# Justin-Huber/SfM-project

Measured on AMD Instinct MI355X. Metric: verified matches/sec (match+RANSAC), higher is better.
Workload: dtype int8 MFMA -> exact int32 (K1), f32 (K2); 1 GPU; cfg4: all 124750 unordered pairs of 500 synthetic images x 4096 128-D u8 SIFT-like descriptors; L2 match (mutual cross check + ratio 4/5) + 8-point RANSAC 4096 hyp/pair (seed 42, Sampson 1 px^2, min 15 inliers); launches of <= 131072 pairs; n_img=500, k=4096, n_hyp=4096, pairs_total=124750, pairs_rank0=124750, launches_rank0=1, parallelism=pair-sharded dp1

## Files before the change

### sfm-project_amd/csrc/match_l2fr.hip

```cpp
#include <algorithm>
#include <climits>
#include <cstdlib>

#include "l2fr_records.h"
#include "match_common.h"

namespace {

typedef int v4i __attribute__((ext_vector_type(4)));
typedef int v16i __attribute__((ext_vector_type(16)));
typedef __attribute__((address_space(3))) void lds_void;
typedef const __attribute__((address_space(1))) void gbl_void;

constexpr int D = 128;
#ifndef L2FR_WAVES
#define L2FR_WAVES 8
#endif
constexpr int WAVES = L2FR_WAVES;
constexpr int SCAN_THREADS = 64 * WAVES;
#ifndef L2FR_QT
#define L2FR_QT 4
#endif
constexpr int QT = L2FR_QT;
constexpr int QB = WAVES * QT * 32;
constexpr int SCAN_MIN_WAVES = 8 / QT;
#ifndef L2FR_CHUNK
#define L2FR_CHUNK 256
#endif
constexpr int CHUNK = L2FR_CHUNK;
constexpr int GROUP = 256;
constexpr int NT = CHUNK / 32;
constexpr int NK = D / 32;
constexpr int SLOTS = D / 16;
constexpr int PIECES = CHUNK * D / 1024 / WAVES;
constexpr int RPP = 1024 / D;
constexpr int KALIGN = CHUNK > GROUP ? CHUNK : GROUP;
constexpr int KMAX = 4096;
constexpr int PAD_INIT = -(1 << 30);
constexpr int E_VALID = l2fr::E_NONE;
static_assert(D == l2fr::REC_D && KMAX == l2fr::REC_KMAX, "l2fr_records.h is sized for D and KMAX");
typedef unsigned long long rec8;

enum : unsigned char { ST_DROP = 0, ST_CAND = 1, ST_SLOW = 2, ST_PASS = 3 };

__device__ __forceinline__ int swz(int row) { return (row >> 1) & 7; }

__device__ __forceinline__ void top2_insert(int& tb, int& ts, int x, int y) {
    const int med = max(min(tb, x), min(max(tb, x), y));
#ifndef L2FR_NO_ASM_MAX3
    int top;
    asm("v_max3_i32 %0, %1, %2, %3" : "=v"(top) : "v"(tb), "v"(x), "v"(y), "v"(med));
#else
    const int top = max(max(x, y), tb);
#endif
    ts = max(ts, med);
    tb = top;
}

__device__ __forceinline__ int dot128(const uint4* x, const uint4* y) {
    int s = 0;
#pragma unroll
    for (int k = 0; k < 8; ++k) {
        const uint4 u = x[k], v = y[k];
        s = __builtin_amdgcn_sdot4((int)u.x, (int)v.x, s, false);
        s = __builtin_amdgcn_sdot4((int)u.y, (int)v.y, s, false);
        s = __builtin_amdgcn_sdot4((int)u.z, (int)v.z, s, false);
        s = __builtin_amdgcn_sdot4((int)u.w, (int)v.w, s, false);
    }
    return s;
}

__device__ __forceinline__ void prep_one(int img, int j, const uint8_t* __restrict__ desc,
                                         const int32_t* __restrict__ n_kp, int k_max, int k_pad,
                                         int32_t* __restrict__ norm, int32_t* __restrict__ cinit,
                                         uint8_t* __restrict__ zero_row,
                                         uint4* __restrict__ desc_i8) {
    if (img == 0 && j < D) zero_row[j] = 0;
    if (j >= k_pad) return;
    int nv = 0;
    if (j < k_max) {
        const uint4* p = (const uint4*)(desc + ((size_t)img * k_max + j) * D);
        uint4* o8 = desc_i8 + ((size_t)img * k_max + j) * SLOTS;
#pragma unroll
        for (int q = 0; q < SLOTS; ++q) {
            const uint4 v = p[q];
            const uint4 x = make_uint4(v.x ^ 0x80808080u, v.y ^ 0x80808080u, v.z ^ 0x80808080u,
                                       v.w ^ 0x80808080u);
            o8[q] = x;
            nv = __builtin_amdgcn_sdot4((int)x.x, (int)x.x, nv, false);
            nv = __builtin_amdgcn_sdot4((int)x.y, (int)x.y, nv, false);
            nv = __builtin_amdgcn_sdot4((int)x.z, (int)x.z, nv, false);
            nv = __builtin_amdgcn_sdot4((int)x.w, (int)x.w, nv, false);
        }
    }
    const size_t o = (size_t)img * k_pad + j;
    norm[o] = nv;
    cinit[o] = (j < n_kp[img]) ? -((nv + 1) >> 1) : PAD_INIT;
}

constexpr int REC_R = 4;

#ifndef L2FR_UNIT
#define L2FR_UNIT 2
#endif
constexpr int UNIT = L2FR_UNIT;
__device__ void build_units(const int32_t* __restrict__ pairs, int n_pairs, int n_img,
                            const int32_t* __restrict__ n_kp, int4* __restrict__ uinfo,
                            int32_t* __restrict__ n_units, int* lds) {
    int* cur = lds;
    int* fu = lds + n_img;
    int* ru = lds + 2 * n_img + 1;
    __shared__ int ftot;
    const int tid = threadIdx.x;
    for (int i = tid; i < n_img; i += 1024) cur[i] = 0;
    __syncthreads();
    auto live = [&](int a, int b) { return n_kp[a] > 0 && n_kp[b] > 0; };
    for (int p = tid; p < n_pairs; p += 1024)
        if (live(pairs[2 * p], pairs[2 * p + 1])) atomicAdd(&cur[pairs[2 * p]], 1);
    __syncthreads();
    if (tid == 0) {
        int f = 0, r = 0;
        for (int i = 0; i < n_img; ++i) {
            const int c = cur[i];
            fu[i] = f;
            ru[i] = r;
            f += c / UNIT;
            r += (c % UNIT) != 0;
            cur[i] = 0;
        }
        fu[n_img] = f;
        ru[n_img] = r;
        ftot = f;
        *n_units = f + r;
    }
    __syncthreads();
    for (int t = tid; t < ru[n_img] * UNIT; t += 1024) uinfo[(size_t)ftot * UNIT + t] = make_int4(-1, 0, 0, 0);
    __syncthreads();
    for (int p = tid; p < n_pairs; p += 1024) {
        const int a = pairs[2 * p], b = pairs[2 * p + 1];
        if (!live(a, b)) continue;
        const int k = atomicAdd(&cur[a], 1);
        const int nf = UNIT * (fu[a + 1] - fu[a]);
        const int u = k < nf ? fu[a] + k / UNIT : ftot + ru[a];
        const int jj = k < nf ? k % UNIT : k - nf;
        uinfo[(size_t)u * UNIT + jj] = jj ? make_int4(p, b, n_kp[b], 0)
                                          : make_int4(p, a, b, n_kp[a] | (n_kp[b] << 16));
    }
}

__device__ void order_block(int ob, const int32_t* __restrict__ pairs, int n_pairs, int n_img,
                            int32_t* __restrict__ order,
                            int2* __restrict__ rng, int32_t* __restrict__ n_rng,
                            const int32_t* __restrict__ n_kp, int4* __restrict__ rinfo,
                            int4* __restrict__ sinfo_f, int unit_blk, int4* __restrict__ uinfo,
                            int32_t* __restrict__ n_units, int* hist) {
    if (ob == unit_blk) {
        build_units(pairs, n_pairs, n_img, n_kp, uinfo, n_units, hist);
        return;
    }
    const int tid = threadIdx.x;
    for (int i = tid; i < n_img; i += 1024) hist[i] = 0;
    __syncthreads();
    for (int p = tid; p < n_pairs; p += 1024) atomicAdd(&hist[pairs[2 * p + 1]], 1);
    __syncthreads();
    int* roff = hist + n_img;
    if (tid == 0) {
        int off = 0, nr = 0;
        for (int i = 0; i < n_img; ++i) {
            const int c = hist[i];
            roff[i] = nr;
            nr += (c + REC_R - 1) / REC_R;
            hist[i] = off;
            off += c;
        }
        n_rng[0] = nr;
        n_rng[1] = 0;
    }
    __syncthreads();
    for (int i = tid; i < n_img; i += 1024) {
        const int c = (i + 1 < n_img ? hist[i + 1] : n_pairs) - hist[i];
        for (int k = 0; k < c; k += REC_R)
            rng[roff[i] + k / REC_R] = make_int2(hist[i] + k, min(REC_R, c - k));
    }
    __syncthreads();
    for (int p = tid; p < n_pairs; p += 1024) {
        const int a = pairs[2 * p], b = pairs[2 * p + 1];
        const int slot = atomicAdd(&hist[b], 1);
        order[slot] = p;
        sinfo_f[slot] = make_int4(p, a, b, n_kp[a] | (n_kp[b] << 16));
    }
    __threadfence_block();
    __syncthreads();
    const int nr = *n_rng;
    for (int r = tid; r < nr; r += 1024) {
        const int2 g = rng[r];
#pragma unroll
        for (int e = 0; e < REC_R; ++e) {
            int4 v = make_int4(-1, 0, 0, 0);
            if (e < g.y) {
                const int p = order[g.x + e], a = pairs[2 * p], b = pairs[2 * p + 1];
                v = make_int4(p, a, b, n_kp[a] | (n_kp[b] << 16));
            }
            rinfo[(size_t)r * REC_R + e] = v;
        }
    }
}

__global__ __launch_bounds__(1024) void l2fr_setup_kernel(
    int n_prep, int bpi, const uint8_t* __restrict__ desc, const int32_t* __restrict__ n_kp,
    int k_max, int k_pad, int32_t* __restrict__ norm, int32_t* __restrict__ cinit,
    uint8_t* __restrict__ zero_row, uint4* __restrict__ desc_i8, const int32_t* __restrict__ pairs,
    int n_pairs, int n_img, int32_t* __restrict__ order_f,
    int2* __restrict__ rng, int32_t* __restrict__ n_rng, int4* __restrict__ rinfo,
    int4* __restrict__ sinfo_f, int unit_blk, int4* __restrict__ uinfo,
    int32_t* __restrict__ n_units) {
    extern __shared__ int hist[];
    const int b = (int)blockIdx.x;
    if (b < n_prep) {
        const int img = b / bpi;
        prep_one(img, (b - img * bpi) * 1024 + (int)threadIdx.x, desc, n_kp, k_max, k_pad, norm,
                 cinit, zero_row, desc_i8);
        return;
    }
    order_block(b - n_prep, pairs, n_pairs, n_img, order_f, rng, n_rng, n_kp, rinfo,
                sinfo_f, unit_blk, uinfo, n_units, hist);
}

__device__ __forceinline__ unsigned char classify(int e1, int e2, long long A, int rnum, int rden,
                                                  long long max_dist) {
    const long long d1lo = max(A - 2LL * e1 - 1, 0LL);
    const long long d2hi = e2 > E_VALID ? A - 2LL * e2 : sfm::DIST_INF;
    if (!sfm::ratio_ok(d1lo, d2hi, rnum, rden, true) || (max_dist >= 0 && !(d1lo < max_dist)))
        return ST_DROP;
    return (e2 == e1) ? ST_SLOW : ST_CAND;
}

struct FwdCls {
    const int32_t* norm;
    int rnum, rden;
    long long max_dist;
    rec8* fwd;
    uint8_t* cls;
};

#ifdef L2FR_CLOCK
constexpr int L2FR_CLOCK_SLOTS = 1 << 16;
constexpr int L2FR_CLOCK_W = 24;
__device__ unsigned long long g_l2fr_clock[L2FR_CLOCK_W * L2FR_CLOCK_SLOTS];
#define L2FR_STAMP(i, v) \
    if (!REV && tid == 0 && bid < L2FR_CLOCK_SLOTS) g_l2fr_clock[L2FR_CLOCK_W * (size_t)bid + (i)] = (v)
#else
#define L2FR_STAMP(i, v)
#endif

template <bool REV>
__device__ __forceinline__ void scan_body(
    const unsigned bid, const unsigned n_bid, const int n_list,
    const uint8_t* __restrict__ desc, const int32_t* __restrict__ n_kp, int k_max, int k_pad,
    const int32_t* __restrict__ cinit, const uint8_t* __restrict__ zero_row,
    const int32_t* __restrict__ pairs, int n_qblk, const int32_t* __restrict__ pair_order,
    const int4* __restrict__ sinfo, int n_blk, const int4* __restrict__ qlist,
    const int32_t* __restrict__ qcount, int4* __restrict__ out, FwdCls fc,
    const int32_t* __restrict__ n_units) {
    __shared__ __attribute__((aligned(16))) unsigned char lds0[CHUNK * D + CHUNK * 4];
    __shared__ __attribute__((aligned(16))) unsigned char lds1[CHUNK * D + CHUNK * 4];

    int p, qi, ti, nq, nb, qb;
    int p2 = -1, ti2 = 0, nb2 = 0;
    int pos = 0, kk = 0;
    if (!REV && n_units) {
        const int nu = *n_units;
        const int u8 = (nu + 7) >> 3;
        const int l = (int)(bid >> 3);
        qb = u8 > 0 ? l / u8 : n_qblk;
        pos = (l - qb * u8) * 8 + (int)(bid & 7);
        if (qb >= n_qblk || pos >= nu) return;
        const int4 u = sinfo[(size_t)UNIT * pos];
        asm volatile("" : : "s"(u.x), "s"(u.y), "s"(u.z), "s"(u.w));
        p = u.x;
        qi = u.y;
        ti = u.z;
        nq = u.w & 0xFFFF;
        nb = u.w >> 16;
    } else if (REV) {
        qb = (int)bid / n_list;
        p = pair_order[(int)bid - qb * n_list];
        qi = pairs[2 * p + 1];
        ti = pairs[2 * p];
        nq = qcount[p];
        nb = n_kp[ti];
    } else {
        const int ppx = (int)(n_bid >> 3) / n_qblk;
        const int l = (int)(bid >> 3);
        const int pos = (int)(bid & 7) * ppx + l % ppx;
        qb = l / ppx;
        if (pos >= n_blk) return;
        const int4 u = sinfo[pos];
        asm volatile("" : : "s"(u.x), "s"(u.y), "s"(u.z), "s"(u.w));
        p = u.x;
        qi = u.y;
        ti = u.z;
        nq = u.w & 0xFFFF;
        nb = u.w >> 16;
    }
    if (qb * QB >= nq || nb <= 0) return;
    const int tid = threadIdx.x, wave = tid >> 6, lane = tid & 63, h = lane >> 5, r32 = lane & 31;
    L2FR_STAMP(0, __builtin_amdgcn_s_memrealtime());

    const uint8_t* db = desc + (size_t)ti * k_max * D;
    const int32_t* cib = cinit + (size_t)ti * k_pad;
    int n_chunk = (nb + CHUNK - 1) / CHUNK;
    const uint8_t* db2 = desc;
    const int32_t* cib2 = cinit;
    auto find_next = [&]() {
        p2 = -1;
        if (REV || !n_units || ++kk >= UNIT) return;
        const int4 v = sinfo[(size_t)UNIT * pos + kk];
        p2 = v.x;
        ti2 = v.y;
        nb2 = v.z;
        db2 = desc + (size_t)ti2 * k_max * D;
        cib2 = cinit + (size_t)ti2 * k_pad;
    };
    find_next();

    auto stage = [&](const uint8_t* sdb, const int32_t* scib, int snb, int ch, unsigned char* dst) {
#pragma unroll
        for (int i = 0; i < PIECES; ++i) {
            const int piece = wave * PIECES + i;
            const int row = piece * RPP + lane / SLOTS;
            const int slot = (lane % SLOTS) ^ swz(row);
            const int j = ch * CHUNK + row;
            const uint8_t* src = (j < snb) ? sdb + (size_t)j * D + slot * 16 : zero_row + slot * 16;
            __builtin_amdgcn_global_load_lds((gbl_void*)src, (lds_void*)(dst + piece * 1024), 16, 0, 0);
        }
        if (tid < CHUNK / 4) {
            const int32_t* src = scib + ch * CHUNK + tid * 4;
            __builtin_amdgcn_global_load_lds((gbl_void*)src, (lds_void*)(dst + CHUNK * D + wave * 1024),
                                             16, 0, 0);
        }
    };
    auto stage_next = [&](int ch, unsigned char* dst) {
        if (ch + 1 < n_chunk) stage(db, cib, nb, ch + 1, dst);
        else if (p2 >= 0) stage(db2, cib2, nb2, 0, dst);
    };

    const int qbase = qb * QB + wave * QT * 32;
    const bool active = qbase < nq;
    const uint8_t* da = desc + (size_t)qi * k_max * D;

    auto emit = [&](int e, int e1, int e2, int t) {
        if (REV) {
            out[(size_t)p * k_pad + e] = make_int4(e1, e2, t, 0);
        } else {
            fc.fwd[(size_t)p * k_pad + e] = l2fr::pack_fwd(e1, e2, t);
            const unsigned char st =
                classify(e1, e2, fc.norm[(size_t)qi * k_pad + e], fc.rnum, fc.rden, fc.max_dist);
            fc.cls[(size_t)p * k_pad + e] =
                st == ST_CAND ? (uint8_t)t : (st == ST_SLOW ? l2fr::CLS_SLOW : l2fr::CLS_DROP);
        }
    };

#if L2FR_MFMA16
    constexpr int QS = 2 * QT;
    const int g4 = lane >> 4, r16 = lane & 15;
    v4i bq[QS][2];
    int tb[QS], ts[QS], t1[QS];
#pragma unroll
    for (int c = 0; c < QS; ++c) {
        const int e = qbase + c * 16 + r16;
        int row = -1;
        if (e < nq) row = REV ? qlist[(size_t)p * k_pad + e].y : e;
        const v4i* src = (const v4i*)((row >= 0) ? da + (size_t)row * D + 32 * g4 : zero_row + 32 * g4);
        bq[c][0] = src[0];
        bq[c][1] = src[1];
        tb[c] = INT_MIN; ts[c] = INT_MIN; t1[c] = 0;
    }
    v4i acc[QS][2];
    auto process = [&](int ch, const unsigned char* cur, unsigned char* nxt) __attribute__((always_inline)) {
        stage_next(ch, nxt);
        const int nt = min(NT, (nb - ch * CHUNK + 31) >> 5);
        if (active) {
            const int* Ci = (const int*)(cur + CHUNK * D);
            auto load_tile = [&](int tt, v4i (&af)[2][2], v4i (&init)[2]) {
#pragma unroll
                for (int u = 0; u < 2; ++u) {
                    const int row = tt * 32 + 16 * u + r16;
                    const int sw = swz(row);
#pragma unroll
                    for (int s = 0; s < 2; ++s)
#ifdef L2FR_ABL_NOLDS
                        af[u][s] = bq[(tt + u + s) & (QS - 1)][s];
#else
                        af[u][s] = *(const v4i*)(cur + row * D + (((2 * g4 + s) ^ sw) << 4));
#endif
#ifdef L2FR_ABL_NOLDS
                    init[u] = v4i{tt, u, tt, u};
#else
                    init[u] = *(const v4i*)(Ci + tt * 32 + 16 * u + 4 * g4);
#endif
                }
            };
            v4i af[2][2], init[2];
            load_tile(0, af, init);
            for (int tt = 0; tt < nt; ++tt) {
                const int gt = ch * NT + tt;
#ifndef L2FR_NO_MPRIO
                __builtin_amdgcn_s_setprio(1);
#endif
#pragma unroll
                for (int s = 0; s < 2; ++s)
#pragma unroll
                    for (int u = 0; u < 2; ++u)
#pragma unroll
                        for (int c = 0; c < QS; ++c)
                            acc[c][u] = __builtin_amdgcn_mfma_i32_16x16x64_i8(
                                af[u][s], bq[c][s], s == 0 ? init[u] : acc[c][u], 0, 0, 0);
#ifndef L2FR_NO_MPRIO
                __builtin_amdgcn_s_setprio(0);
#endif
                if (tt + 1 < nt) load_tile(tt + 1, af, init);
#pragma unroll
                for (int c = 0; c < QS; ++c) {
                    const int o = tb[c];
#ifdef L2FR_ABL_NOEPI
                    tb[c] = max(tb[c], acc[c][0][0] ^ acc[c][1][3]);
#else
#pragma unroll
                    for (int u = 0; u < 2; ++u) {
                        top2_insert(tb[c], ts[c], acc[c][u][0], acc[c][u][1]);
                        top2_insert(tb[c], ts[c], acc[c][u][2], acc[c][u][3]);
                    }
#endif
                    t1[c] = (tb[c] != o) ? gt : t1[c];
                }
            }
        }
    };
#else
    v4i bq[QT][NK];
    int tb[QT], ts[QT], t1[QT];
#pragma unroll
    for (int c = 0; c < QT; ++c) {
        const int e = qbase + c * 32 + r32;
        int row = -1;
        if (e < nq) row = REV ? qlist[(size_t)p * k_pad + e].y : e;
        const v4i* src = (const v4i*)((row >= 0) ? da + (size_t)row * D + (D / 2) * h
                                                 : zero_row + (D / 2) * h);
#pragma unroll
        for (int s = 0; s < NK; ++s) bq[c][s] = src[s];
        tb[c] = INT_MIN; ts[c] = INT_MIN; t1[c] = 0;
    }

    v16i acc[QT];
    auto epi_all = [&](int gt) {
#pragma unroll
        for (int u = 0; u < QT; ++u) {
            const int o = tb[u];
#ifdef L2FR_ABL_NOEPI
            tb[u] = max(tb[u], acc[u][0] ^ acc[u][15]);
#else
#pragma unroll
            for (int r = 0; r < 16; r += 2) top2_insert(tb[u], ts[u], acc[u][r], acc[u][r + 1]);
#endif
            t1[u] = (tb[u] != o) ? gt : t1[u];
        }
    };

    auto process = [&](int ch, const unsigned char* cur, unsigned char* nxt) __attribute__((always_inline)) {
        stage_next(ch, nxt);
        const int nt = min(NT, (nb - ch * CHUNK + 31) >> 5);
        if (active) {
            const int* Ci = (const int*)(cur + CHUNK * D);
            auto load_tile = [&](int tt, v4i (&af)[NK], v16i& init) {
                const int row = tt * 32 + r32;
                const int sw = swz(row);
#pragma unroll
                for (int s = 0; s < NK; ++s)
#ifdef L2FR_ABL_NOLDS
                    af[s] = bq[(tt + s) & (QT - 1)][s];
#else
                    af[s] = *(const v4i*)(cur + row * D + ((((SLOTS / 2) * h + s) ^ sw) << 4));
#endif
#pragma unroll
                for (int g = 0; g < 4; ++g) {
#ifdef L2FR_ABL_NOLDS
                    const v4i cv = v4i{tt, g, tt, g};
#else
                    const v4i cv = *(const v4i*)(Ci + tt * 32 + 8 * g + 4 * h);
#endif
                    init[4 * g + 0] = cv.x; init[4 * g + 1] = cv.y;
                    init[4 * g + 2] = cv.z; init[4 * g + 3] = cv.w;
                }
            };
            v4i af[NK];
            v16i init;
            load_tile(0, af, init);
            for (int tt = 0; tt < nt; ++tt) {
                const int gt = ch * NT + tt;
#ifndef L2FR_NO_MPRIO
                __builtin_amdgcn_s_setprio(1);
#endif
#pragma unroll
                for (int s = 0; s < NK; ++s)
#pragma unroll
                    for (int c = 0; c < QT; ++c)
                        acc[c] = __builtin_amdgcn_mfma_i32_32x32x32_i8(af[s], bq[c][s],
                                                                        s == 0 ? init : acc[c], 0, 0, 0);
#ifndef L2FR_NO_MPRIO
                __builtin_amdgcn_s_setprio(0);
#endif
                if (tt + 1 < nt) load_tile(tt + 1, af, init);
                epi_all(gt);
            }
        }
    };
#endif

    auto epilogue = [&]() {
#if L2FR_MFMA16
#pragma unroll
        for (int c = 0; c < QS; ++c) {
            int e1 = tb[c], e2 = ts[c], t = t1[c];
#pragma unroll
            for (int m = 16; m <= 32; m <<= 1) {
                const int P1 = __shfl_xor(e1, m), P2 = __shfl_xor(e2, m), PT = __shfl_xor(t, m);
                e2 = max(min(e1, P1), max(e2, P2));
                t = e1 > P1 ? t : (P1 > e1 ? PT : min(t, PT));
                e1 = max(e1, P1);
            }
            const int e = qbase + c * 16 + r16;
            if (g4 == 0 && e < nq) emit(e, e1, e2, t);
            tb[c] = INT_MIN; ts[c] = INT_MIN; t1[c] = 0;
        }
#else
#pragma unroll
        for (int c = 0; c < QT; ++c) {
            const int P1 = __shfl_xor(tb[c], 32), P2 = __shfl_xor(ts[c], 32),
                      PT = __shfl_xor(t1[c], 32);
            const int e1 = max(tb[c], P1);
            const int e2 = max(min(tb[c], P1), max(ts[c], P2));
            const int t = tb[c] > P1 ? t1[c] : (P1 > tb[c] ? PT : min(t1[c], PT));
            const int e = qbase + c * 32 + r32;
            if (h == 0 && e < nq) emit(e, e1, e2, t);
            tb[c] = INT_MIN; ts[c] = INT_MIN; t1[c] = 0;
        }
#endif
    };

    if (n_chunk > 0) stage(db, cib, nb, 0, lds0);
    __syncthreads();
    L2FR_STAMP(1, __builtin_amdgcn_s_memrealtime());
    L2FR_STAMP(2, __builtin_amdgcn_s_memtime());
    auto run_pair = [&](unsigned char* s0, unsigned char* s1) __attribute__((always_inline)) {
        for (int ch = 0; ch < n_chunk; ch += 2) {
            process(ch, s0, s1);
            __syncthreads();
            if (ch < 16) L2FR_STAMP(3 + ch, __builtin_amdgcn_s_memrealtime());
            if (ch + 1 < n_chunk) process(ch + 1, s1, s0);
            __syncthreads();
            if (ch + 1 < 16) L2FR_STAMP(4 + ch, __builtin_amdgcn_s_memrealtime());
        }
    };
    int g = 0;
    for (;;) {
        if (g & 1)
            run_pair(lds1, lds0);
        else
            run_pair(lds0, lds1);
        g += n_chunk;
        L2FR_STAMP(19, __builtin_amdgcn_s_memtime());
        L2FR_STAMP(20, __builtin_amdgcn_s_memrealtime());
        if (active) epilogue();
        if (p2 < 0) break;
        p = p2;
        ti = ti2;
        nb = nb2;
        db = db2;
        cib = cib2;
        n_chunk = (nb + CHUNK - 1) / CHUNK;
        find_next();
    }
#ifdef L2FR_CLOCK
    L2FR_STAMP(21, __builtin_amdgcn_s_memrealtime());
    L2FR_STAMP(22, (unsigned)__builtin_amdgcn_s_getreg((31 << 11) | 4));
    L2FR_STAMP(23, (unsigned)__builtin_amdgcn_s_getreg((15 << 11) | 20));
#endif
}

__global__ __launch_bounds__(SCAN_THREADS, SCAN_MIN_WAVES) void l2fr_scan_fwd_kernel(
    const uint8_t* __restrict__ desc, const int32_t* __restrict__ n_kp, int k_max, int k_pad,
    const int32_t* __restrict__ cinit, const uint8_t* __restrict__ zero_row,
    const int32_t* __restrict__ pairs, int n_qblk, const int4* __restrict__ sinfo, int n_blk,
    FwdCls fc, const int32_t* __restrict__ n_units) {
    scan_body<false>(blockIdx.x, gridDim.x, 0, desc, n_kp, k_max, k_pad, cinit, zero_row, pairs, n_qblk,
                     nullptr, sinfo, n_blk, nullptr, nullptr, nullptr, fc, n_units);
}

constexpr int REV_GRID = 1024;
__global__ __launch_bounds__(SCAN_THREADS, SCAN_MIN_WAVES) void l2fr_scan_rev_kernel(
    const uint8_t* __restrict__ desc, const int32_t* __restrict__ n_kp, int k_max, int k_pad,
    const int32_t* __restrict__ cinit, const uint8_t* __restrict__ zero_row,
    const int32_t* __restrict__ pairs, int n_qblk, const int32_t* __restrict__ flist,
    const int32_t* __restrict__ n_flag, const int4* __restrict__ qlist,
    const int32_t* __restrict__ qcount, int4* __restrict__ out) {
    const int nl = *n_flag;
    for (unsigned u = blockIdx.x; u < (unsigned)(nl * n_qblk); u += gridDim.x) {
        scan_body<true>(u, 0, nl, desc, n_kp, k_max, k_pad, cinit, zero_row, pairs, n_qblk, flist,
                        nullptr, 0, qlist, qcount, out, FwdCls{}, nullptr);
        __syncthreads();
    }
}

struct Top2 { long long b1; int j1; long long b2; };

__device__ __forceinline__ Top2 top2_merge(Top2 x, Top2 y) {
    const bool xf = (x.b1 < y.b1) || (x.b1 == y.b1 && x.j1 < y.j1);
    Top2 r;
    r.b1 = xf ? x.b1 : y.b1;
    r.j1 = xf ? x.j1 : y.j1;
    r.b2 = min(min(x.b2, y.b2), xf ? y.b1 : x.b1);
    return r;
}

__device__ Top2 exact_row_scan(const uint4* qrow, const uint8_t* db, const int32_t* normb, int nb,
                               int qnorm, Top2* red) {
    const int tid = threadIdx.x;
    uint4 x[SLOTS];
#pragma unroll
    for (int s = 0; s < SLOTS; ++s) x[s] = qrow[s];
    Top2 m{sfm::DIST_INF, INT_MAX, sfm::DIST_INF};
    for (int j = tid; j < nb; j += 256) {
        const int dot = dot128(x, (const uint4*)(db + (size_t)j * D));
        const long long d = (long long)qnorm + normb[j] - 2LL * dot;
        m = top2_merge(m, Top2{d, j, sfm::DIST_INF});
    }
    red[tid] = m;
    __syncthreads();
    for (int s = 128; s > 0; s >>= 1) {
        if (tid < s) red[tid] = top2_merge(red[tid], red[tid + s]);
        __syncthreads();
    }
    const Top2 r = red[0];
    __syncthreads();
    return r;
}

__device__ __forceinline__ int compact_rec(bool keep, int4 rec, int base, int* wsum, int4* dst) {
    const int tid = threadIdx.x, lane = tid & 63, wave = tid >> 6;
    const unsigned long long bal = __ballot(keep);
    const int pre = __popcll(bal & ((1ull << lane) - 1ull));
    if (lane == 0) wsum[wave] = __popcll(bal);
    __syncthreads();
    int off = 0, tot = 0;
    for (int w = 0; w < 4; ++w) {
        const int s = wsum[w];
        off += (w < wave) ? s : 0;
        tot += s;
    }
    if (keep) dst[base + off + pre] = rec;
    __syncthreads();
    return base + tot;
}

#ifndef L2FR_REC_SB
#define L2FR_REC_SB 2
#endif
constexpr int REC_SB = L2FR_REC_SB;
__global__ __launch_bounds__(256, REC_SB > 2 ? 2 : 3) void l2fr_recover_mfma_kernel(
    const uint8_t* __restrict__ desc, int k_max, int k_pad, const int32_t* __restrict__ norm,
    const int32_t* __restrict__ cinit, const int4* __restrict__ rinfo,
    const int32_t* __restrict__ n_rng, const rec8* __restrict__ fwd,
    const uint8_t* __restrict__ cls, int rnum, int rden, long long max_dist,
    rec8* __restrict__ qst) {
    __shared__ unsigned short clist[REC_R * KMAX];
    __shared__ __attribute__((aligned(16))) int gini[GROUP];
    __shared__ unsigned char gpar[GROUP];
    __shared__ unsigned long long wlo[4], whi[4];
    __shared__ int toff[9];
    const int ngrp = k_pad / GROUP;
    const int ri = (int)(blockIdx.x / ngrp), grp = (int)(blockIdx.x % ngrp), tid = threadIdx.x;
    if (ri >= *n_rng) return;
    const int wave = tid >> 6, lane = tid & 63, h = lane >> 5, r32 = lane & 31;
    int4 pi[REC_R];
#pragma unroll
    for (int e = 0; e < REC_R; ++e) pi[e] = rinfo[(size_t)ri * REC_R + e];
    const int b = pi[0].z, nb = pi[0].w >> 16;
    const int ntiles = (nb + 31) >> 5, tg = grp * 8;
    if (nb <= 0 || tg >= ntiles) return;
    const uint8_t* db = desc + (size_t)b * k_max * D;

    uint4 cv[REC_R];
#pragma unroll
    for (int e = 0; e < REC_R; ++e) {
        cv[e] = make_uint4(0xFFFFFFFFu, 0xFFFFFFFFu, 0xFFFFFFFFu, 0xFFFFFFFFu);
        if (pi[e].x >= 0 && tid * 16 < (pi[e].w & 0xFFFF))
            cv[e] = ((const uint4*)(cls + (size_t)pi[e].x * k_pad))[tid];
    }
    v4i af[2][NK];
#pragma unroll
    for (int u = 0; u < 2; ++u) {
        const int row = (tg + 2 * wave + u) * 32 + r32;
#pragma unroll
        for (int s = 0; s < NK; ++s)
            af[u][s] = row < nb ? *(const v4i*)(db + (size_t)row * D + 64 * h + 16 * s) : v4i{0, 0, 0, 0};
    }
    {
        const size_t o = (size_t)b * k_pad + tg * 32 + tid;
        gini[tid] = cinit[o];
        gpar[tid] = (unsigned char)(norm[o] & 1);
    }
    unsigned msk[REC_R];
    unsigned long long lo = 0, hi = 0;
    const unsigned g8 = 0x01010101u * ((unsigned)grp << 3);
#pragma unroll
    for (int e = 0; e < REC_R; ++e) {
        const int na = pi[e].x >= 0 ? (pi[e].w & 0xFFFF) : 0;
        const unsigned cw[4] = {cv[e].x, cv[e].y, cv[e].z, cv[e].w};
        unsigned m = 0;
#pragma unroll
        for (int k = 0; k < 4; ++k) {
            const unsigned t = (cw[k] ^ g8) & 0xF8F8F8F8u;
            const unsigned nz = ((t & 0x7F7F7F7Fu) + 0x7F7F7F7Fu) | t;
            const unsigned z = ~nz & 0x80808080u;
            m |= (((z >> 7) & 1u) | ((z >> 14) & 2u) | ((z >> 21) & 4u) | ((z >> 28) & 8u)) << (4 * k);
        }
        const int lim = na - tid * 16;
        m &= lim >= 16 ? 0xFFFFu : (lim <= 0 ? 0u : (1u << lim) - 1u);
        msk[e] = m;
        for (unsigned mm = m; mm; mm &= mm - 1) {
            const int k = __builtin_ctz(mm);
            const unsigned c = (cw[k >> 2] >> (8 * (k & 3))) & 7u;
            const unsigned long long one = 1ull << (16 * (c & 3));
            if (c & 4) hi += one; else lo += one;
        }
    }
    unsigned long long plo = lo, phi = hi;
#pragma unroll
    for (int d = 1; d < 64; d <<= 1) {
        const unsigned long long vl = __shfl_up(plo, d), vh = __shfl_up(phi, d);
        if (lane >= d) { plo += vl; phi += vh; }
    }
    if (lane == 63) { wlo[wave] = plo; whi[wave] = phi; }
    __syncthreads();
    unsigned long long blo = 0, bhi = 0, tlo = 0, thi = 0;
#pragma unroll
    for (int w = 0; w < 4; ++w) {
        blo += w < wave ? wlo[w] : 0ull;
        bhi += w < wave ? whi[w] : 0ull;
        tlo += wlo[w];
        thi += whi[w];
    }
    unsigned long long slo = 0, shi = 0;
    {
        int o = 0;
#pragma unroll
        for (int t = 0; t < 8; ++t) {
            const unsigned long long tot = t < 4 ? tlo : thi, bef = t < 4 ? blo : bhi,
                                     mine = t < 4 ? plo - lo : phi - hi;
            const int sh = 16 * (t & 3);
            const unsigned long long v =
                (unsigned long long)(o + (int)((bef >> sh) & 0xFFFF) + (int)((mine >> sh) & 0xFFFF)) << sh;
// ... 347 lines not shown
#pragma unroll
    for (int i = 0; i < TAIL_NQ; ++i) {
        const int4 w4 = *(const int4*)wcnt[i];
        const int ww[4] = {w4.x, w4.y, w4.z, w4.w};
        int off = M;
#pragma unroll
        for (int w = 0; w < 4; ++w) {
            off += w < wave ? ww[w] : 0;
            M += ww[w];
        }
        const unsigned long long bal = __ballot((outm >> i) & 1u);
        if ((outm >> i) & 1u) {
            const int o = off + __popcll(bal & ((1ull << lane) - 1ull));
            const l2fr::Res r = l2fr::unpack_res(raw[i]);
            om[2 * o] = i * 256 + tid;
            om[2 * o + 1] = r.j1;
            od[o] = r.d1;
        }
    }
    if (tid == 0) {
        out_count[p] = M;
        if (stats) atomicAdd(&stats[0], 1ull);
    }
}

__global__ __launch_bounds__(256) void l2fr_final_kernel(
    const uint8_t* __restrict__ desc, const int32_t* __restrict__ n_kp, int k_max, int k_pad,
    const int32_t* __restrict__ norm, const int32_t* __restrict__ cinit,
    const int32_t* __restrict__ pairs, const int4* __restrict__ surv,
    const int32_t* __restrict__ scount, const int4* __restrict__ rev,
    const int32_t* __restrict__ flist, const int32_t* __restrict__ n_flag,
    int32_t* __restrict__ out_count, int32_t* __restrict__ out_match,
    int32_t* __restrict__ out_dist) {
    __shared__ int wsum[8];
    __shared__ int amb[256];
    __shared__ int namb;
    __shared__ unsigned char keepx[256];
    __shared__ long long redd[256];
    __shared__ int redq[256];
    const int tid = threadIdx.x, nl = *n_flag;
    for (int li = blockIdx.x; li < nl; li += gridDim.x) {
    const int p = flist[li];
    const int a = pairs[2 * p], b = pairs[2 * p + 1];
    const int na = n_kp[a];
    const int S = scount[p];
    const int4* sv = surv + (size_t)p * k_pad;
    const int4* rv = rev + (size_t)p * k_pad;
    const int32_t* na_norm = norm + (size_t)a * k_pad;
    const int32_t* nb_norm = norm + (size_t)b * k_pad;
    const int32_t* ca = cinit + (size_t)a * k_pad;
    const uint8_t* da = desc + (size_t)a * k_max * D;
    const uint4* dbv = (const uint4*)(desc + (size_t)b * k_max * D);
    int32_t* om = out_match + (size_t)p * k_max * 2;
    int32_t* od = out_dist + (size_t)p * k_max;
    int base = 0;
    for (int k0 = 0; k0 < S; k0 += 256) {
        const int k = k0 + tid;
        int4 s = make_int4(0, 0, 0, 0);
        bool keep = false;
        if (tid == 0) namb = 0;
        __syncthreads();
        if (k < S) {
            s = sv[k];
            const int4 r = rv[k];
            const int dot = (int)(((long long)na_norm[s.x] + nb_norm[s.y] - s.z) >> 1);
            const int ep = dot + ca[s.x];
            keep = (ep == r.x) && (r.y < r.x);
            if (ep == r.x && r.y == r.x) amb[atomicAdd(&namb, 1)] = tid;
        }
        keepx[tid] = keep;
        __syncthreads();
        const int nam = namb;
        for (int i = 0; i < nam; ++i) {
            const int who = amb[i];
            const int4 e = sv[k0 + who];
            uint4 y[SLOTS];
#pragma unroll
            for (int u = 0; u < SLOTS; ++u) y[u] = dbv[(size_t)e.y * SLOTS + u];
            long long bd = sfm::DIST_INF;
            int bq = INT_MAX;
            for (int q = tid; q < na; q += 256) {
                const int dot = dot128((const uint4*)(da + (size_t)q * D), y);
                const long long d = (long long)na_norm[q] + nb_norm[e.y] - 2LL * dot;
                if (d < bd) { bd = d; bq = q; }
            }
            redd[tid] = bd; redq[tid] = bq;
            __syncthreads();
            for (int st = 128; st > 0; st >>= 1) {
                if (tid < st) {
                    const long long od2 = redd[tid + st];
                    const int oq = redq[tid + st];
                    if (od2 < redd[tid] || (od2 == redd[tid] && oq < redq[tid])) {
                        redd[tid] = od2; redq[tid] = oq;
                    }
                }
                __syncthreads();
            }
            if (tid == 0) keepx[who] = (redq[0] == e.x);
            __syncthreads();
        }
        keep = keepx[tid] != 0 && k < S;
        base = sfm::compact256(keep, s.x, s.y, s.z, base, wsum, om, od);
    }
    if (tid == 0) out_count[p] = base;
    }
}

__global__ void l2fr_dump_kernel(const int32_t* __restrict__ n_kp, const int32_t* __restrict__ pairs,
                                 int k_max, int k_pad, const int4* __restrict__ rec,
                                 const rec8* __restrict__ fwd8,
                                 const int32_t* __restrict__ cnt, int32_t* __restrict__ out_count,
                                 int32_t* __restrict__ out_match, int32_t* __restrict__ out_dist) {
    const int p = blockIdx.x;
    const int n = cnt ? cnt[p] : n_kp[pairs[2 * p]];
    for (int i = threadIdx.x; i < n; i += blockDim.x) {
        int4 r;
        if (rec) {
            r = rec[(size_t)p * k_pad + i];
        } else {
            const l2fr::Fwd f = l2fr::unpack_fwd(fwd8[(size_t)p * k_pad + i]);
            r = make_int4(f.e1, f.e2, f.tile, 0);
        }
        out_match[((size_t)p * k_max + i) * 2] = r.x;
        out_match[((size_t)p * k_max + i) * 2 + 1] = r.y;
        out_dist[(size_t)p * k_max + i] = r.z;
    }
    if (threadIdx.x == 0) out_count[p] = n;
}

}

int sfm_match_l2fr_launch(sfm_ctx* ctx, const uint8_t* desc, const int32_t* n_kp, int32_t n_img,
                          int32_t k_max, const int32_t* pairs, int32_t n_pairs,
                          const sfm_match_params* prm, int32_t* out_count, int32_t* out_match,
                          int32_t* out_dist) {
    hipStream_t st = ctx->stream;
    if (k_max == 0) {
        SFM_HIP_CHECK(hipMemsetAsync(out_count, 0, sizeof(int32_t) * n_pairs, st));
        return SFM_OK;
    }
    const int k_pad = (int)sfm::align_up((size_t)k_max, KALIGN);
    SFM_REQUIRE(k_pad <= KMAX, "sfm_match_batch: L2 matcher needs k_max <= 4096");
    const int n_qblk = (k_max + QB - 1) / QB;
    const size_t tab = (size_t)n_img * k_pad * sizeof(int32_t);
    const size_t recb = (size_t)n_pairs * k_pad * sizeof(int4);
    const size_t cntb = sfm::align_up(sizeof(int32_t) * (size_t)n_pairs, 256);
    const size_t descb = sfm::align_up((size_t)n_img * k_max * D, 256);
    const size_t ordb = sfm::align_up(sizeof(int32_t) * (size_t)n_pairs, 256);
    const size_t clsb = sfm::align_up((size_t)n_pairs * k_pad, 256);
    const int n_rng_max = n_pairs / REC_R + n_img + 1;
    const size_t rngb = sfm::align_up(sizeof(int2) * (size_t)n_rng_max, 256);
    const size_t rinfob = sizeof(int4) * (size_t)n_rng_max * REC_R;
    const size_t sinfob = sfm::align_up(sizeof(int4) * (size_t)n_pairs, 256);
    const size_t uinfob = sfm::align_up(UNIT * sizeof(int4) * (size_t)n_pairs, 256);
    char* ws = (char*)sfm::workspace(ctx, 256 + 2 * tab + 2 * recb + cntb + descb + ordb + clsb +
                                              256 + rngb + rinfob + 256 + sinfob + uinfob + 256 +
                                              cntb);
    if (!ws) return SFM_ERR_NOMEM;
    char* w = ws;
    uint8_t* zero_row = (uint8_t*)w; w += 256;
    int32_t* norm = (int32_t*)w; w += tab;
    int32_t* cinit = (int32_t*)w; w += tab;
    int4* surv = (int4*)w; w += recb;
    int4* rev = (int4*)w; w += recb;
    rec8* fwd = (rec8*)rev;
    rec8* qst = fwd + (size_t)n_pairs * k_pad;
    int32_t* scount = (int32_t*)w; w += cntb;
    uint8_t* desc_i8 = (uint8_t*)w; w += descb;
    int32_t* ord_f = (int32_t*)w; w += ordb;
    uint8_t* cls = (uint8_t*)w; w += clsb;
    int32_t* n_rng = (int32_t*)w; w += 256;
    int32_t* n_flag = n_rng + 1;
    int2* rng = (int2*)w; w += rngb;
    int4* rinfo = (int4*)w; w += rinfob;
    int4* sinfo_f = (int4*)sfm::align_up((size_t)w, 256);
    int4* uinfo = (int4*)((char*)sinfo_f + sinfob);
    int32_t* n_units = (int32_t*)((char*)uinfo + uinfob);
    int32_t* flist = (int32_t*)((char*)n_units + 256);
    static const bool units_env = [] {
        const char* e = getenv("SFM_L2FR_UNITS");
        return !(e && e[0] == '0');
    }();
    const bool units = units_env && (3 * (size_t)n_img + 2) * sizeof(int) <= 65536;
    const int ppx = (n_pairs + 7) / 8;
    const int n_blk = n_pairs;
    const int grid = 8 * ppx * n_qblk;
    const bool mutual = prm->cross_check == SFM_XC_MUTUAL;

    const int unit_blk = units ? 1 : -1;
    const int bpi = (k_pad + 1023) / 1024, n_prep = bpi * n_img;
    hipLaunchKernelGGL(l2fr_setup_kernel, dim3(n_prep + 1 + (units ? 1 : 0)), dim3(1024),
                       ((units ? 3 : 2) * (size_t)n_img + 2) * sizeof(int), st, n_prep, bpi, desc, n_kp,
                       k_max, k_pad, norm, cinit, zero_row, (uint4*)desc_i8, pairs, n_pairs, n_img,
                       ord_f, rng, n_rng, rinfo, sinfo_f, unit_blk, uinfo, n_units);
    SFM_HIP_CHECK(hipGetLastError());
    const FwdCls fc{norm, prm->ratio_num, prm->ratio_den, (long long)prm->max_dist, fwd, cls};
    hipLaunchKernelGGL(l2fr_scan_fwd_kernel, dim3(grid), dim3(SCAN_THREADS), 0, st, desc_i8, n_kp, k_max,
                       k_pad, cinit, zero_row, pairs, n_qblk, (const int4*)(units ? uinfo : sinfo_f),
                       n_blk, fc, (const int32_t*)(units ? n_units : nullptr));
    SFM_HIP_CHECK(hipGetLastError());
    const char* dbg = getenv("SFM_L2FR_DEBUG");
    int dmode = dbg ? atoi(dbg) : 0;
    if (dmode < 1 || dmode > 3) dmode = 0;
    if (dmode == 1) {
        hipLaunchKernelGGL(l2fr_dump_kernel, dim3(n_pairs), dim3(256), 0, st, n_kp, pairs, k_max,
                           k_pad, (const int4*)nullptr, (const rec8*)fwd, (const int32_t*)nullptr,
                           out_count, out_match, out_dist);
        return SFM_OK;
    }
    hipLaunchKernelGGL(l2fr_recover_mfma_kernel, dim3(n_rng_max * (k_pad / GROUP)), dim3(256), 0, st,
                       desc_i8, k_max, k_pad, norm, cinit, (const int4*)rinfo, (const int32_t*)n_rng,
                       (const rec8*)fwd, (const uint8_t*)cls, prm->ratio_num, prm->ratio_den,
                       (long long)prm->max_dist, qst);
    SFM_HIP_CHECK(hipGetLastError());
    const char* ce = getenv("SFM_L2FR_CERT");
    const bool cert = mutual && dmode == 0 && !(ce && ce[0] == '0');
    const char* cc = getenv("SFM_L2FR_CERT_CAP");
    const long long cap = cc ? atoll(cc) : CERT_CAP_DEFAULT;
    unsigned long long* stats = cert && ctx->cert_stats ? ctx->cert_acc : nullptr;
    if (stats)
        SFM_HIP_CHECK(hipMemsetAsync(stats, 0, 3 * sizeof(unsigned long long), st));
    auto tail = !mutual && dmode == 0 ? l2fr_tail_kernel<TAIL_DIRECT>
                : cert                ? l2fr_tail_kernel<TAIL_CERT>
                                      : l2fr_tail_kernel<TAIL_SPILL>;
    hipLaunchKernelGGL(tail, dim3(n_pairs), dim3(256), 0, st, desc_i8, n_kp, k_max, k_pad, norm, pairs,
                       (const rec8*)fwd, (const uint8_t*)cls, qst, prm->ratio_num, prm->ratio_den,
                       (long long)prm->max_dist, cap, surv, scount, flist, n_flag, stats, out_count,
                       out_match, out_dist);
    SFM_HIP_CHECK(hipGetLastError());
    if (!mutual && dmode == 0) return SFM_OK;
    if (dmode == 2) {
        hipLaunchKernelGGL(l2fr_dump_kernel, dim3(n_pairs), dim3(256), 0, st, n_kp, pairs, k_max,
                           k_pad, (const int4*)surv, (const rec8*)nullptr, (const int32_t*)scount,
                           out_count, out_match, out_dist);
        return SFM_OK;
    }
    if (mutual) {
        hipLaunchKernelGGL(l2fr_scan_rev_kernel, dim3(REV_GRID), dim3(SCAN_THREADS), 0, st, desc_i8, n_kp,
                           k_max, k_pad, cinit, zero_row, pairs, n_qblk, (const int32_t*)flist,
                           (const int32_t*)n_flag, (const int4*)surv, (const int32_t*)scount, rev);
        SFM_HIP_CHECK(hipGetLastError());
    }
    if (dmode == 3) {
        hipLaunchKernelGGL(l2fr_dump_kernel, dim3(n_pairs), dim3(256), 0, st, n_kp, pairs, k_max,
                           k_pad, (const int4*)rev, (const rec8*)nullptr, (const int32_t*)scount,
                           out_count, out_match, out_dist);
        return SFM_OK;
    }
    hipLaunchKernelGGL(l2fr_final_kernel, dim3(REV_GRID), dim3(256), 0, st, desc_i8, n_kp, k_max, k_pad,
                       norm, cinit, pairs, surv, scount, rev, (const int32_t*)flist,
                       (const int32_t*)n_flag, out_count, out_match, out_dist);
    SFM_HIP_CHECK(hipGetLastError());
    return SFM_OK;
}

extern "C" int32_t sfm_l2fr_rev_grid(void) { return REV_GRID; }

extern "C" int sfm_match_cert_stats(sfm_ctx* ctx, int32_t enable, uint64_t* out) {
    SFM_REQUIRE(ctx, "sfm_match_cert_stats: ctx is NULL");
    SFM_HIP_CHECK(hipSetDevice(ctx->device));
    if (!ctx->cert_acc) {
        SFM_HIP_CHECK(hipMalloc(&ctx->cert_acc, 3 * sizeof(unsigned long long)));
        SFM_HIP_CHECK(hipMemsetAsync(ctx->cert_acc, 0, 3 * sizeof(unsigned long long), ctx->stream));
    }
    if (out) {
        unsigned long long h[3];
        SFM_HIP_CHECK(hipMemcpyAsync(h, ctx->cert_acc, sizeof(h), hipMemcpyDeviceToHost, ctx->stream));
        SFM_HIP_CHECK(hipStreamSynchronize(ctx->stream));
        out[0] = h[0]; out[1] = h[1]; out[2] = h[2];
    }
    ctx->cert_stats = enable ? 1 : 0;
    return SFM_OK;
}

#ifdef L2FR_CLOCK
extern "C" int sfm_debug_l2fr_stamps(unsigned long long* host, int32_t n_blocks) {
    const size_t n = L2FR_CLOCK_W * (size_t)std::min(n_blocks, L2FR_CLOCK_SLOTS);
    SFM_HIP_CHECK(hipDeviceSynchronize());
    SFM_HIP_CHECK(hipMemcpyFromSymbol(host, HIP_SYMBOL(g_l2fr_clock), n * sizeof(unsigned long long)));
    return SFM_OK;
}
#endif
```

Before: 272.6 million verified matches/s.

## Pick pair-unit size at runtime, shrink scan grid, and stage query norms in LDS

Makes the number of pairs grouped per scan block a runtime value. A heuristic picks 8, 4 or 2 from pairs, images, query blocks and CU count, and an env var can override it. The forward scan grid is now sized to the unit bound instead of one block per pair, which cuts idle early-exit blocks. The epilogue loads query norms into LDS with global_load_lds and spreads emit work across all lanes instead of half. Larger units reuse the query tile across more pairs but can reduce parallelism and add per-block serial work.

```diff
diff --git a/sfm-project_amd/csrc/l2fr_units.h b/sfm-project_amd/csrc/l2fr_units.h
--- /dev/null
+++ b/sfm-project_amd/csrc/l2fr_units.h
@@ -0,0 +1,41 @@
+#pragma once
+#include <cstdint>
+
+#if defined(__HIPCC__)
+#define L2FR_UNITS_HD __host__ __device__ inline __attribute__((always_inline))
+#else
+#define L2FR_UNITS_HD inline
+#endif
+
+namespace l2fr {
+
+constexpr int UNIT_MAX = 8;
+
+L2FR_UNITS_HD bool unit_supported(int u) { return u == 1 || u == 2 || u == 3 || u == 4 || u == 8; }
+
+L2FR_UNITS_HD long long unit_bound(long long n_pairs, long long n_img, int u) {
+    const long long b = n_pairs / u + n_img;
+    return b < n_pairs ? b : n_pairs;
+}
+
+L2FR_UNITS_HD long long unit_records_max(long long n_pairs, long long n_img) {
+    return n_pairs + UNIT_MAX * (n_img < n_pairs ? n_img : n_pairs);
+}
+
+L2FR_UNITS_HD long long unit_grid(long long bound, int n_qblk) {
+    return 8 * ((bound + 7) / 8) * n_qblk;
+}
+
+L2FR_UNITS_HD double unit_rounds(long long n_pairs, long long n_img, int n_qblk, int n_cu, int u) {
+    return (double)(unit_bound(n_pairs, n_img, u) * n_qblk) / (double)(n_cu > 0 ? n_cu : 1);
+}
+
+constexpr double UNIT_R_MIN = 250.0;
+
+L2FR_UNITS_HD int unit_pick(long long n_pairs, long long n_img, int n_qblk, int n_cu) {
+    if (unit_rounds(n_pairs, n_img, n_qblk, n_cu, 8) >= UNIT_R_MIN) return 8;
+    if (unit_rounds(n_pairs, n_img, n_qblk, n_cu, 4) >= UNIT_R_MIN) return 4;
+    return 2;
+}
+
+}
diff --git a/sfm-project_amd/csrc/match_l2fr.hip b/sfm-project_amd/csrc/match_l2fr.hip
--- a/sfm-project_amd/csrc/match_l2fr.hip
+++ b/sfm-project_amd/csrc/match_l2fr.hip
@@ -3,6 +3,7 @@
 #include <cstdlib>
 
 #include "l2fr_records.h"
+#include "l2fr_units.h"
 #include "match_common.h"
 
 namespace {
@@ -104,8 +105,9 @@
 #define L2FR_UNIT 2
 #endif
 constexpr int UNIT = L2FR_UNIT;
+static_assert(UNIT == 1 || UNIT == 2 || UNIT == 3 || UNIT == 4 || UNIT == 8, "unsupported L2FR_UNIT");
 __device__ void build_units(const int32_t* __restrict__ pairs, int n_pairs, int n_img,
-                            const int32_t* __restrict__ n_kp, int4* __restrict__ uinfo,
+                            const int32_t* __restrict__ n_kp, int unit, int4* __restrict__ uinfo,
                             int32_t* __restrict__ n_units, int* lds) {
     int* cur = lds;
     int* fu = lds + n_img;
@@ -124,8 +126,8 @@
             const int c = cur[i];
             fu[i] = f;
             ru[i] = r;
-            f += c / UNIT;
-            r += (c % UNIT) != 0;
+            f += c / unit;
+            r += (c % unit) != 0;
             cur[i] = 0;
         }
         fu[n_img] = f;
@@ -134,16 +136,16 @@
         *n_units = f + r;
     }
     __syncthreads();
-    for (int t = tid; t < ru[n_img] * UNIT; t += 1024) uinfo[(size_t)ftot * UNIT + t] = make_int4(-1, 0, 0, 0);
+    for (int t = tid; t < ru[n_img] * unit; t += 1024) uinfo[(size_t)ftot * unit + t] = make_int4(-1, 0, 0, 0);
     __syncthreads();
     for (int p = tid; p < n_pairs; p += 1024) {
         const int a = pairs[2 * p], b = pairs[2 * p + 1];
         if (!live(a, b)) continue;
         const int k = atomicAdd(&cur[a], 1);
-        const int nf = UNIT * (fu[a + 1] - fu[a]);
-        const int u = k < nf ? fu[a] + k / UNIT : ftot + ru[a];
-        const int jj = k < nf ? k % UNIT : k - nf;
-        uinfo[(size_t)u * UNIT + jj] = jj ? make_int4(p, b, n_kp[b], 0)
+        const int nf = unit * (fu[a + 1] - fu[a]);
+        const int u = k < nf ? fu[a] + k / unit : ftot + ru[a];
+        const int jj = k < nf ? k % unit : k - nf;
+        uinfo[(size_t)u * unit + jj] = jj ? make_int4(p, b, n_kp[b], 0)
                                           : make_int4(p, a, b, n_kp[a] | (n_kp[b] << 16));
     }
 }
@@ -152,10 +154,10 @@
                             int32_t* __restrict__ order,
                             int2* __restrict__ rng, int32_t* __restrict__ n_rng,
                             const int32_t* __restrict__ n_kp, int4* __restrict__ rinfo,
-                            int4* __restrict__ sinfo_f, int unit_blk, int4* __restrict__ uinfo,
-                            int32_t* __restrict__ n_units, int* hist) {
+                            int4* __restrict__ sinfo_f, int unit_blk, int unit,
+                            int4* __restrict__ uinfo, int32_t* __restrict__ n_units, int* hist) {
     if (ob == unit_blk) {
-        build_units(pairs, n_pairs, n_img, n_kp, uinfo, n_units, hist);
+        build_units(pairs, n_pairs, n_img, n_kp, unit, uinfo, n_units, hist);
         return;
     }
     const int tid = threadIdx.x;
@@ -212,7 +214,7 @@
     uint8_t* __restrict__ zero_row, uint4* __restrict__ desc_i8, const int32_t* __restrict__ pairs,
     int n_pairs, int n_img, int32_t* __restrict__ order_f,
     int2* __restrict__ rng, int32_t* __restrict__ n_rng, int4* __restrict__ rinfo,
-    int4* __restrict__ sinfo_f, int unit_blk, int4* __restrict__ uinfo,
+    int4* __restrict__ sinfo_f, int unit_blk, int unit, int4* __restrict__ uinfo,
     int32_t* __restrict__ n_units) {
     extern __shared__ int hist[];
     const int b = (int)blockIdx.x;
@@ -223,7 +225,7 @@
         return;
     }
     order_block(b - n_prep, pairs, n_pairs, n_img, order_f, rng, n_rng, n_kp, rinfo,
-                sinfo_f, unit_blk, uinfo, n_units, hist);
+                sinfo_f, unit_blk, unit, uinfo, n_units, hist);
 }
 
 __device__ __forceinline__ unsigned char classify(int e1, int e2, long long A, int rnum, int rden,
@@ -261,9 +263,11 @@
     const int32_t* __restrict__ pairs, int n_qblk, const int32_t* __restrict__ pair_order,
     const int4* __restrict__ sinfo, int n_blk, const int4* __restrict__ qlist,
     const int32_t* __restrict__ qcount, int4* __restrict__ out, FwdCls fc,
-    const int32_t* __restrict__ n_units) {
+    const int32_t* __restrict__ n_units, const int unit) {
     __shared__ __attribute__((aligned(16))) unsigned char lds0[CHUNK * D + CHUNK * 4];
     __shared__ __attribute__((aligned(16))) unsigned char lds1[CHUNK * D + CHUNK * 4];
+    __shared__ __attribute__((aligned(16))) int lnorm[REV ? 4 : QB];
+    (void)lnorm;
 
     int p, qi, ti, nq, nb, qb;
     int p2 = -1, ti2 = 0, nb2 = 0;
@@ -275,7 +279,7 @@
         qb = u8 > 0 ? l / u8 : n_qblk;
         pos = (l - qb * u8) * 8 + (int)(bid & 7);
         if (qb >= n_qblk || pos >= nu) return;
-        const int4 u = sinfo[(size_t)UNIT * pos];
+        const int4 u = sinfo[(size_t)unit * pos];
         asm volatile("" : : "s"(u.x), "s"(u.y), "s"(u.z), "s"(u.w));
         p = u.x;
         qi = u.y;
@@ -314,8 +318,8 @@
     const int32_t* cib2 = cinit;
     auto find_next = [&]() {
         p2 = -1;
-        if (REV || !n_units || ++kk >= UNIT) return;
-        const int4 v = sinfo[(size_t)UNIT * pos + kk];
+        if (REV || !n_units || ++kk >= unit) return;
+        const int4 v = sinfo[(size_t)unit * pos + kk];
         p2 = v.x;
         ti2 = v.y;
         nb2 = v.z;
@@ -354,8 +358,12 @@
             out[(size_t)p * k_pad + e] = make_int4(e1, e2, t, 0);
         } else {
             fc.fwd[(size_t)p * k_pad + e] = l2fr::pack_fwd(e1, e2, t);
-            const unsigned char st =
-                classify(e1, e2, fc.norm[(size_t)qi * k_pad + e], fc.rnum, fc.rden, fc.max_dist);
+#ifdef L2FR_ABL_EPI
+            const int A = fc.norm[(size_t)qi * k_pad + e];
+#else
+            const int A = lnorm[e - qb * QB];
+#endif
+            const unsigned char st = classify(e1, e2, A, fc.rnum, fc.rden, fc.max_dist);
             fc.cls[(size_t)p * k_pad + e] =
                 st == ST_CAND ? (uint8_t)t : (st == ST_SLOW ? l2fr::CLS_SLOW : l2fr::CLS_DROP);
         }
@@ -519,6 +527,7 @@
 
     auto epilogue = [&]() {
 #if L2FR_MFMA16
+        int m1[QS], m2[QS], mt[QS];
 #pragma unroll
         for (int c = 0; c < QS; ++c) {
             int e1 = tb[c], e2 = ts[c], t = t1[c];
@@ -529,25 +538,72 @@
                 t = e1 > P1 ? t : (P1 > e1 ? PT : min(t, PT));
                 e1 = max(e1, P1);
             }
+            m1[c] = e1; m2[c] = e2; mt[c] = t;
+            tb[c] = INT_MIN; ts[c] = INT_MIN; t1[c] = 0;
+        }
+#ifdef L2FR_ABL_EPI
+#pragma unroll
+        for (int c = 0; c < QS; ++c) {
             const int e = qbase + c * 16 + r16;
-            if (g4 == 0 && e < nq) emit(e, e1, e2, t);
-            tb[c] = INT_MIN; ts[c] = INT_MIN; t1[c] = 0;
+            if (g4 == 0 && e < nq) emit(e, m1[c], m2[c], mt[c]);
         }
 #else
+        constexpr int PG = QS / 4;
+        int ln = lane;
+        asm volatile("" : "+v"(ln));
+        const int eg = ln >> 4;
+#pragma unroll
+        for (int k = 0; k < PG; ++k) {
+            int e1 = m1[k], e2 = m2[k], t = mt[k];
+#pragma unroll
+            for (int g = 1; g < 4; ++g) {
+                e1 = eg == g ? m1[g * PG + k] : e1;
+                e2 = eg == g ? m2[g * PG + k] : e2;
+                t = eg == g ? mt[g * PG + k] : t;
+            }
+            const int e = qbase + (eg * PG + k) * 16 + (ln & 15);
+            if (e < nq) emit(e, e1, e2, t);
+        }
+#endif
+#else
+        int m1[QT], m2[QT], mt[QT];
 #pragma unroll
         for (int c = 0; c < QT; ++c) {
             const int P1 = __shfl_xor(tb[c], 32), P2 = __shfl_xor(ts[c], 32),
                       PT = __shfl_xor(t1[c], 32);
-            const int e1 = max(tb[c], P1);
-            const int e2 = max(min(tb[c], P1), max(ts[c], P2));
-            const int t = tb[c] > P1 ? t1[c] : (P1 > tb[c] ? PT : min(t1[c], PT));
+            m1[c] = max(tb[c], P1);
+            m2[c] = max(min(tb[c], P1), max(ts[c], P2));
+            mt[c] = tb[c] > P1 ? t1[c] : (P1 > tb[c] ? PT : min(t1[c], PT));
+            tb[c] = INT_MIN; ts[c] = INT_MIN; t1[c] = 0;
+        }
+#ifdef L2FR_ABL_EPI
+#pragma unroll
+        for (int c = 0; c < QT; ++c) {
             const int e = qbase + c * 32 + r32;
-            if (h == 0 && e < nq) emit(e, e1, e2, t);
-            tb[c] = INT_MIN; ts[c] = INT_MIN; t1[c] = 0;
-        }
+            if (h == 0 && e < nq) emit(e, m1[c], m2[c], mt[c]);
+        }
+#else
+        constexpr int PG = QT / 2;
+        int ln = lane;
+        asm volatile("" : "+v"(ln));
+        const int eh = ln >> 5;
+#pragma unroll
+        for (int k = 0; k < PG; ++k) {
+            const int e = qbase + (eh * PG + k) * 32 + (ln & 31);
+            if (e < nq)
+                emit(e, eh ? m1[PG + k] : m1[k], eh ? m2[PG + k] : m2[k], eh ? mt[PG + k] : mt[k]);
+        }
+#endif
 #endif
     };
 
+#ifndef L2FR_ABL_EPI
+    if (!REV && tid < QB / 4) {
+        const int r0 = min(qb * QB + tid * 4, k_pad - 4);
+        __builtin_amdgcn_global_load_lds((gbl_void*)(fc.norm + (size_t)qi * k_pad + r0),
+                                         (lds_void*)((unsigned char*)lnorm + wave * 1024), 16, 0, 0);
+    }
+#endif
     if (n_chunk > 0) stage(db, cib, nb, 0, lds0);
     __syncthreads();
     L2FR_STAMP(1, __builtin_amdgcn_s_memrealtime());
@@ -592,9 +648,9 @@
     const uint8_t* __restrict__ desc, const int32_t* __restrict__ n_kp, int k_max, int k_pad,
     const int32_t* __restrict__ cinit, const uint8_t* __restrict__ zero_row,
     const int32_t* __restrict__ pairs, int n_qblk, const int4* __restrict__ sinfo, int n_blk,
-    FwdCls fc, const int32_t* __restrict__ n_units) {
+    FwdCls fc, const int32_t* __restrict__ n_units, int unit) {
     scan_body<false>(blockIdx.x, gridDim.x, 0, desc, n_kp, k_max, k_pad, cinit, zero_row, pairs, n_qblk,
-                     nullptr, sinfo, n_blk, nullptr, nullptr, nullptr, fc, n_units);
+                     nullptr, sinfo, n_blk, nullptr, nullptr, nullptr, fc, n_units, unit);
 }
 
 constexpr int REV_GRID = 1024;
@@ -607,7 +663,7 @@
     const int nl = *n_flag;
     for (unsigned u = blockIdx.x; u < (unsigned)(nl * n_qblk); u += gridDim.x) {
         scan_body<true>(u, 0, nl, desc, n_kp, k_max, k_pad, cinit, zero_row, pairs, n_qblk, flist,
-                        nullptr, 0, qlist, qcount, out, FwdCls{}, nullptr);
+                        nullptr, 0, qlist, qcount, out, FwdCls{}, nullptr, 1);
         __syncthreads();
     }
 }
@@ -1261,7 +1317,8 @@
     const size_t rngb = sfm::align_up(sizeof(int2) * (size_t)n_rng_max, 256);
     const size_t rinfob = sizeof(int4) * (size_t)n_rng_max * REC_R;
     const size_t sinfob = sfm::align_up(sizeof(int4) * (size_t)n_pairs, 256);
-    const size_t uinfob = sfm::align_up(UNIT * sizeof(int4) * (size_t)n_pairs, 256);
+    const size_t uinfob =
+        sfm::align_up(sizeof(int4) * (size_t)l2fr::unit_records_max(n_pairs, n_img), 256);
     char* ws = (char*)sfm::workspace(ctx, 256 + 2 * tab + 2 * recb + cntb + descb + ordb + clsb +
                                               256 + rngb + rinfob + 256 + sinfob + uinfob + 256 +
                                               cntb);
@@ -1286,14 +1343,25 @@
     int4* uinfo = (int4*)((char*)sinfo_f + sinfob);
     int32_t* n_units = (int32_t*)((char*)uinfo + uinfob);
     int32_t* flist = (int32_t*)((char*)n_units + 256);
-    static const bool units_env = [] {
-        const char* e = getenv("SFM_L2FR_UNITS");
-        return !(e && e[0] == '0');
-    }();
+    const char* ue = getenv("SFM_L2FR_UNITS");
+    const bool units_env = !(ue && ue[0] == '0');
     const bool units = units_env && (3 * (size_t)n_img + 2) * sizeof(int) <= 65536;
+    const int picked = l2fr::unit_pick(n_pairs, n_img, n_qblk, ctx->n_cu);
+    int unit = picked > 2 ? picked : UNIT;
+    if (const char* fe = getenv("SFM_L2FR_UNIT")) {
+        unit = atoi(fe);
+        SFM_REQUIRE(l2fr::unit_supported(unit), "sfm_match_batch: SFM_L2FR_UNIT must be 1, 2, 3, 4 or 8");
+    }
+    const int n_blk = n_pairs;
     const int ppx = (n_pairs + 7) / 8;
-    const int n_blk = n_pairs;
-    const int grid = 8 * ppx * n_qblk;
+#ifdef L2FR_ABL_GRID
+    const long long ubound = n_pairs;
+#else
+    const long long ubound = l2fr::unit_bound(n_pairs, n_img, unit);
+#endif
+    const long long grid_ll = units ? l2fr::unit_grid(ubound, n_qblk) : 8LL * ppx * n_qblk;
+    SFM_REQUIRE(grid_ll <= INT_MAX, "sfm_match_batch: too many pairs for one forward scan");
+    const int grid = (int)grid_ll;
     const bool mutual = prm->cross_check == SFM_XC_MUTUAL;
 
     const int unit_blk = units ? 1 : -1;
@@ -1301,12 +1369,12 @@
     hipLaunchKernelGGL(l2fr_setup_kernel, dim3(n_prep + 1 + (units ? 1 : 0)), dim3(1024),
                        ((units ? 3 : 2) * (size_t)n_img + 2) * sizeof(int), st, n_prep, bpi, desc, n_kp,
                        k_max, k_pad, norm, cinit, zero_row, (uint4*)desc_i8, pairs, n_pairs, n_img,
-                       ord_f, rng, n_rng, rinfo, sinfo_f, unit_blk, uinfo, n_units);
+                       ord_f, rng, n_rng, rinfo, sinfo_f, unit_blk, unit, uinfo, n_units);
     SFM_HIP_CHECK(hipGetLastError());
     const FwdCls fc{norm, prm->ratio_num, prm->ratio_den, (long long)prm->max_dist, fwd, cls};
     hipLaunchKernelGGL(l2fr_scan_fwd_kernel, dim3(grid), dim3(SCAN_THREADS), 0, st, desc_i8, n_kp, k_max,
                        k_pad, cinit, zero_row, pairs, n_qblk, (const int4*)(units ? uinfo : sinfo_f),
-                       n_blk, fc, (const int32_t*)(units ? n_units : nullptr));
+                       n_blk, fc, (const int32_t*)(units ? n_units : nullptr), unit);
     SFM_HIP_CHECK(hipGetLastError());
     const char* dbg = getenv("SFM_L2FR_DEBUG");
     int dmode = dbg ? atoi(dbg) : 0;
```

Result: no change. 273.7 million verified matches/s, median of 6 (+0.4%).
